# NVlabs/ODISE

Hardware: AMD Instinct MI355X
Metric: panoptic-inference images/sec @1024x1024 (higher is better)
Workload: dtype f16

## Files before the change

### include/odise_hip_tools.h

```cpp
#ifndef ODISE_HIP_TOOLS_H
#define ODISE_HIP_TOOLS_H

#include "odise_hip.h"

#ifdef __cplusplus
extern "C" {
#endif

int odise_hip_sizeof_gemm_desc(void);
int odise_hip_sizeof_conv_desc(void);
int odise_hip_sizeof_attn_desc(void);
int odise_hip_sizeof_post_desc(void);
int odise_hip_sizeof_infer_desc(void);

int odise_hip_gemm_forced(odise_hip_ctx* ctx, const odise_gemm_desc* d, int tile, int splitk);
int odise_hip_conv2d_forced(odise_hip_ctx* ctx, const odise_conv_desc* d, int tile, int splitk);
int odise_hip_last_tile(void);
int odise_hip_gemm_ln(odise_hip_ctx* ctx, const odise_gemm_desc* d, const float* part, int parts, float inv_c, float eps, const float* colsum,
                      float* final_out, const float* fin, const float* rowsum, float* stats_out);
int odise_hip_conv2d_gn_forced(odise_hip_ctx* ctx, const odise_conv_desc* d, int tile, int splitk, const float* gamma, const float* beta,
                               int groups, float eps, int act, void* y_norm, float* stats_scratch, int* stats_blocks);
int odise_hip_gemm_debug(int flags);

int odise_hip_post_generic(int on);
int odise_hip_sem_tile(int tile);
int odise_hip_gn_tuning(int chunk_factor, int fold_in_apply);
int odise_hip_msda_unfused(int on);
int odise_hip_msda_fused_forward(odise_hip_ctx* ctx, const void* value, const float* off, const float* aw, const int* hs3, const int* ws3, int B, int M, int fused,
                                 void* out, float* loc_scratch, float* w_scratch);

int odise_hip_stage_timeline(odise_hip_ctx* ctx, int on);
int odise_hip_stage_timeline_read(odise_hip_ctx* ctx, char* names, int names_cap, float* gpu_ms, double* host_ms, int cap, int* n);

int odise_hip_prefetch_stats(odise_hip_ctx* ctx, int* enqueued, int* hits, int* dropped, int* failed);

int odise_hip_launch_log(odise_hip_ctx* ctx, int on);
int odise_hip_launch_log_read(odise_hip_ctx* ctx, int* out6, int cap, int* n);

int odise_hip_set_lanes(odise_hip_ctx* ctx, int lanes);

int odise_hip_backbone_maps(odise_hip_ctx* ctx, float** out4, int* shape_bchw4x4);

int odise_hip_mfma_probe(odise_hip_ctx* ctx, float* host_out);

int odise_hip_maskclip_token_mask(odise_hip_ctx* ctx, const void* logits_f16, void* out_u8, int B, int Q, int h, int w, int S, int patch, int T,
                                  int64_t ldm, int plain);
#ifdef __cplusplus
}
#endif
#endif
```

### odise_amd/csrc/engine.cpp

```cpp
#include <stdlib.h>

#include "engine.h"

#include <string.h>

namespace odise {

void unet_destroy(ModelStore* ms);
void extractor_destroy(ModelStore* ms);
void maskgen_destroy(ModelStore* ms);
void classify_destroy(ModelStore* ms);

ModelStore* store_of(odise_hip_ctx* ctx) {
    if (!ctx->models) ctx->models = new ModelStore();
    return (ModelStore*)ctx->models;
}

void free_allocs(std::vector<void*>& owned) {
    if (owned.empty()) return;
    (void)hipDeviceSynchronize();
    for (void* p : owned) (void)hipFree(p);
    owned.clear();
}

// ... 195 lines not shown
    if (x.c != w.cin_pad) {
        set_error("conv: input has %d channels, weight expects %d", x.c, w.cin_pad);
        return ODISE_ERR_ARG;
    }
    if (pad < 0) pad = w.k / 2;
    if (pad_t < 0) pad_t = pad;
    if (pad_l < 0) pad_l = pad;
    const int hin = upsample ? 2 * x.h : x.h, win = upsample ? 2 * x.w : x.w;
    if (oh < 0) oh = (hin + 2 * pad - w.k) / stride + 1;
    if (ow < 0) ow = (win + 2 * pad - w.k) / stride + 1;
    if (!y.p) ODISE_TRY(alloc(y, x.n, oh, ow, w.cout));
    odise_conv_desc d;
    memset(&d, 0, sizeof(d));
    d.N = x.n; d.H = x.h; d.W = x.w; d.Cin = x.c;
    d.Cout = w.cout; d.KH = w.k; d.KW = w.k; d.stride = stride; d.pad_t = pad_t; d.pad_l = pad_l; d.OH = oh; d.OW = ow;
    d.upsample2x = upsample ? 1 : 0;
    d.X = x.p; d.Wt = w.w; d.Y = y.p; d.y_dtype = ODISE_F16;
    d.bias = w.b;
    d.residual = residual ? residual->p : nullptr;
    d.per_image_add = per_image_add;
    d.per_image_add_ld = pia_ld;
    d.act = act;
    ms->macs += (double)x.n * oh * ow * w.cout * w.k * w.k * w.cin;
    y.gn_blocks = 0;
#ifdef ODISE_TOOLS
    if (y.gn_part && getenv("ODISE_NO_GN_FUSION")) return odise_hip_conv2d(ctx, &d);
#endif
    if (y.gn_part) return conv_forced(ctx, &d, -1, 0, y.gn_part, &y.gn_blocks);
    return odise_hip_conv2d(ctx, &d);
}

int Exec::alloc_gn_stats(Act& a) {
    const int64_t blocks = ceil_div((int64_t)a.h * a.w, 64);
    a.gn_part = (float*)alloc_bytes((size_t)a.n * blocks * a.c * 2 * sizeof(float));
    a.gn_blocks = 0;
    return a.gn_part ? ODISE_OK : ODISE_ERR_NOMEM;
}

int Exec::linear(const f16* x, int64_t M, const LinW& w, f16* y, int act, const f16* residual, bool geglu) {
    odise_gemm_desc d;
    memset(&d, 0, sizeof(d));
    d.M = (int)M; d.N = w.out; d.K = w.in;
    d.A = x; d.lda = w.in;
    d.W = w.w; d.ldw = w.in;
    d.C = y; d.ldc = geglu ? w.out / 2 : w.out; d.c_dtype = ODISE_F16;
    d.bias_n = w.b;
    d.residual = residual; d.ldr = d.ldc;
    d.act = act; d.geglu = geglu ? 1 : 0; d.alpha = 1.f; d.batch = 1;
    return gemm(d);
}

int Exec::group_norm(const Act& x, const NormW& w, Act& y, float eps, int act) {
    if (!y.p) ODISE_TRY(alloc(y, x.n, x.h, x.w, x.c));
    if (x.gn_part && x.gn_blocks > 0)
        return group_norm_from_colpart(ctx, x.p, y.p, w.g, w.b, x.n, x.h * x.w, x.c, 32, eps, act, x.gn_part, x.gn_blocks);
    return odise_hip_group_norm(ctx, x.p, y.p, w.g, w.b, x.n, x.h * x.w, x.c, 32, eps, act);
}

int Exec::layer_norm(const f16* x, f16* y, int64_t rows, const NormW& w, float eps) {
    return odise_hip_layer_norm(ctx, x, y, w.g, w.b, (int)rows, w.c, eps);
}

}

using namespace odise;

extern "C" int odise_hip_load_weight(odise_hip_ctx* ctx, const char* name, const float* host_data, const int64_t* shape, int ndim) {
    ODISE_REQUIRE(ctx && name && host_data && (ndim == 0 || shape), "load_weight: null argument");
    ODISE_REQUIRE(ndim >= 0 && ndim <= 4, "load_weight: rank %d not in [0,4]", ndim);
    ModelStore* ms = store_of(ctx);
    HostTensor t;
    int64_t n = 1;
    for (int i = 0; i < ndim; ++i) {
        ODISE_REQUIRE(shape[i] >= 0, "load_weight: negative dim");
        t.shape.push_back(shape[i]);
        n *= shape[i];
    }
    t.data.assign(host_data, host_data + n);
    ms->host[std::string(name)] = std::move(t);
    return ODISE_OK;
}

extern "C" int odise_hip_clear_host_weights(odise_hip_ctx* ctx) {
    ODISE_REQUIRE(ctx, "clear_host_weights: null context");
    store_of(ctx)->host.clear();
    return ODISE_OK;
}
```

### odise_amd/csrc/engine.h

```cpp
#pragma once
#include <map>
#include <utility>
#include <string>
#include <vector>

#include "common.h"

namespace odise {

struct HostTensor {
    std::vector<float> data;
    std::vector<int64_t> shape;
    int64_t numel() const {
        int64_t n = 1;
        for (auto s : shape) n *= s;
        return n;
    }
};

struct Arena {
    char* base = nullptr;
    size_t cap = 0, off = 0, peak = 0;
    void* alloc(size_t bytes) {
        off = (off + 255) & ~(size_t)255;
// ... 34 lines not shown
};

struct UNetModel;

struct EncoderOut {
    Act tap0, tap1;
    Act xt, zdec;
};
struct PrefetchKey {
    int B = 0, layout = 0;
    std::vector<const void*> images;
    std::vector<int> hw;
    bool operator==(const PrefetchKey& o) const { return B == o.B && layout == o.layout && images == o.images && hw == o.hw; }
};
struct Prefetch {
    bool has_pending = false, has_ready = false;
    PrefetchKey pending, ready;
    int ready_slot = 0;
    EncoderOut out;
    int crops = 0;
    bool use_now = false;
    int n_enqueued = 0, n_hits = 0, n_dropped = 0, n_failed = 0;
    Arena arena[2];
};

struct ClipKV {
    void* buf = nullptr;
    size_t cap = 0;
    f16* qk = nullptr;
    f16* vt = nullptr;
    f16* cls = nullptr;
    int B = 0, TP = 0, layers = 0, width = 0;
    size_t qk_stride = 0, vt_stride = 0;
    int64_t ldvt = 0;
    const float* plan_image = nullptr;
    int plan_B = 0, plan_H = 0, plan_W = 0;
    bool planned = false, ready = false, on_lane2 = false;
};

struct ModelStore {
    std::map<std::string, HostTensor> host;
    std::vector<void*> dev_allocs;
    std::vector<void*>* alloc_sink = nullptr;
    void track(void* p) { (alloc_sink ? *alloc_sink : dev_allocs).push_back(p); }
    Arena arena;
    Arena arena2;
    Prefetch pf;
    ClipKV mclip;
    UNetModel* unet = nullptr;
    struct ExtractorModel* extractor = nullptr;
    struct MaskGenModel* maskgen = nullptr;
    struct ClassifyModel* classify = nullptr;
    double macs = 0.0;
};

ModelStore* store_of(odise_hip_ctx* ctx);
struct AllocScope {
    ModelStore* ms;
    std::vector<void*>* prev;
    AllocScope(ModelStore* m, std::vector<void*>& owned) : ms(m), prev(m->alloc_sink) { m->alloc_sink = &owned; }
    ~AllocScope() { ms->alloc_sink = prev; }
};
void free_allocs(std::vector<void*>& owned);

struct Packer {
    odise_hip_ctx* ctx;
    ModelStore* ms;
    std::string prefix;
    std::string missing;

    const HostTensor* find(const std::string& key);
    int upload(const void* host, size_t bytes, void** dev);
    int conv(const std::string& key, ConvW& out, bool bias = true);
    int linear(const std::string& key, LinW& out, bool bias = true);
    int norm(const std::string& key, NormW& out);
    int vec_f32(const std::string& key, float** out, int64_t expect);
};

struct Exec {
    odise_hip_ctx* ctx;
    ModelStore* ms;
    int alloc(Act& a, int n, int h, int w, int c);
    int alloc_gn_stats(Act& a);
    void* alloc_bytes(size_t bytes);

    int conv(const Act& x, const ConvW& w, Act& y, int stride = 1, int pad = -1, bool upsample = false, const Act* residual = nullptr,
             const float* per_image_add = nullptr, int64_t pia_ld = 0, int act = ODISE_ACT_NONE, int pad_t = -1, int pad_l = -1,
             int oh = -1, int ow = -1);
    int linear(const f16* x, int64_t M, const LinW& w, f16* y, int act = ODISE_ACT_NONE, const f16* residual = nullptr,
               bool geglu = false);
    int group_norm(const Act& x, const NormW& w, Act& y, float eps, int act);
    int layer_norm(const f16* x, f16* y, int64_t rows, const NormW& w, float eps);
    int gemm(const odise_gemm_desc& d);
    int attention(const odise_attn_desc& d);
};


int ensure_lane2(odise_hip_ctx* ctx, ModelStore* ms, size_t arena_bytes);
struct Lane2 {
    odise_hip_ctx* ctx;
    ModelStore* ms;
    hipStream_t s0;
    void* w0;
    Lane2(odise_hip_ctx* c, ModelStore* m) : ctx(c), ms(m), s0(c->stream), w0(c->ws) {
        ctx->stream = ctx->stream2;
        ctx->ws = ctx->ws2;
// ... 137 lines not shown
```

### odise_amd/csrc/gemm.hip

```cpp
#include "common.h"
#include <stdlib.h>
#include <type_traits>

#ifdef ODISE_TOOLS
#define ODISE_ABLATE(g, bit) ((g).dbg & (bit))
#else
#define ODISE_ABLATE(g, bit) false
#endif

namespace odise {

struct GemmEpi {
    void* C;
    int64_t ldc;
    int c_dtype;
    const float* bias_n;
    const float* bias_m;
    const float* scale_m;
    const f16* residual;
    int64_t ldr;
    const float* rowgroup_add;
    int rows_per_group;
    int64_t ldg;
    int act;
// ... 771 lines not shown
        }
        __syncthreads();
        if (stats) {
            float* red = reinterpret_cast<float*>(smem);
            if (lane < CHW) {
#pragma unroll
                for (int i = 0; i < 8; ++i) {
                    red[((wm * BN) + wn * WTN + lane * 8 + i) * 2 + 0] = s8[i];
                    red[((wm * BN) + wn * WTN + lane * 8 + i) * 2 + 1] = q8[i];
                }
            }
            __syncthreads();
            for (int c = threadIdx.x; c < BN; c += 64 * NWAVES) {
                float a = 0.f, bb = 0.f;
                for (int r = 0; r < WAVES_M; ++r) { a += red[(r * BN + c) * 2]; bb += red[(r * BN + c) * 2 + 1]; }
                if (n0 + c < g.N) {
                    float* o = e.gn_stats + ((int64_t)(m0 / BM) * g.N + n0 + c) * 2;
                    o[0] = a;
                    o[1] = bb;
                }
            }
        }
    }
}

template <int BM, int BN, int WAVES_M, int WAVES_N, int WG, bool HALO = false, bool STATS = false, bool PAIRS = true, int EW16 = 0, bool GEGLU_OK = false, int LDSB = 0>
__device__ __forceinline__ void gemm_epilogue(const GemmArgs& g, WaveAcc<BM, BN, WAVES_M, WAVES_N>& acc, char* smem, int m0, int n0, int z, int zb, bool split) {
    using FL = FragLayout;
    if constexpr (LDSB > 0 && WAVES_M * WAVES_N == 8 && (64 % ((BN / WAVES_N) / 8)) == 0) {
        if (g.epi.fast && !split && !g.epi.geglu && !g.epi_block && !ODISE_ABLATE(g, 8)) {
            gemm_epilogue_wave<BM, BN, WAVES_M, WAVES_N, HALO, STATS, GEGLU_OK, LDSB>(g, acc, smem, m0, n0, zb);
            return;
        }
    }
    if constexpr (EW16 > 0) {
        if (g.epi.f16path && !split && !ODISE_ABLATE(g, 8)) {
            if constexpr (GEGLU_OK) {
                if (g.epi.geglu) { gemm_epilogue_f16<BM, BN, WAVES_M, WAVES_N, EW16, HALO, false, true>(g, acc, smem, m0, n0, zb); return; }
            }
            if (!g.epi.geglu) { gemm_epilogue_f16<BM, BN, WAVES_M, WAVES_N, EW16, HALO, STATS, false>(g, acc, smem, m0, n0, zb); return; }
        }
    }
    constexpr int NT = 64 * WAVES_M * WAVES_N;
    constexpr int WTM = BM / WAVES_M, WTN = BN / WAVES_N;
    constexpr int TM = WTM / 32, TN = WTN / 32;
    constexpr int ROWS = WG * WTM;
    const int tid = threadIdx.x;
    const int lane = tid & 63;
    const int wave = tid >> 6;
    const int wm = wave / WAVES_N, wn = wave % WAVES_N;
    constexpr int LDS_LD = BN + 4;
    constexpr int CH = BN / 8;
    float* stg = reinterpret_cast<float*>(smem);
    const bool stats = STATS && (NT % CH == 0) && g.epi.gn_stats != nullptr && !split;
    float s8[8], q8[8];
#pragma unroll
    for (int i = 0; i < 8; ++i) s8[i] = q8[i] = 0.f;
    constexpr int LPR = (BN * 2 + 127) / 128;
    constexpr int NPF = (BM * LPR + NT - 1) / NT;
    unsigned pf[NPF];
    const bool prefetch = g.epi.residual != nullptr && !split && !ODISE_ABLATE(g, 64);
    if (prefetch) {
#pragma unroll
        for (int i = 0; i < NPF; ++i) {
            const int li = tid + i * NT;
            const int rt = li / LPR, seg = li - rt * LPR;
            int m = m0 + rt;
            if (HALO) {
                const int patch = m0 / BM;
                const int per_img = g.cg.halo_tx * g.cg.halo_ty;
                const int img = patch / per_img, pr = patch - img * per_img;
                const int oy = (pr / g.cg.halo_tx) * 16 + (rt >> 4), ox = (pr % g.cg.halo_tx) * 16 + (rt & 15);
                m = (oy < g.cg.OH && ox < g.cg.OW) ? (img * g.cg.OH + oy) * g.cg.OW + ox : g.M;
            }
            pf[i] = 0u;
            if (rt < BM && m < g.M && n0 + seg * 64 + 2 <= g.N)
                pf[i] = *reinterpret_cast<const unsigned*>(g.epi.residual + (int64_t)zb * g.epi.strideR + (int64_t)m * g.epi.ldr + n0 + seg * 64);
        }
        asm volatile("" ::: "memory");
    }
#pragma unroll
    for (int gp = 0; gp < WAVES_M / WG; ++gp) {
        if (gp > 0) lds_barrier();
        if (wm / WG == gp) {
#pragma unroll
            for (int p = 0; p < TM; ++p)
#pragma unroll
                for (int j = 0; j < TN; ++j) {
#pragma unroll
                    for (int rr = 0; rr < FL::NR; ++rr) {
                        const int row = (wm % WG) * WTM + p * 32 + FL::row(lane, rr);
#pragma unroll
                        for (int q = 0; q < FL::NC; ++q) {
                            const int col = wn * WTN + j * 32 + FL::col(lane, q);
                            const int r0 = 4 * (rr * FL::NC + q);
                            *reinterpret_cast<float4*>(&stg[row * LDS_LD + col]) =
                                make_float4(acc_get(acc, p, j, r0), acc_get(acc, p, j, r0 + 1), acc_get(acc, p, j, r0 + 2), acc_get(acc, p, j, r0 + 3));
                        }
                    }
                }
        }
        lds_barrier();
        if (gp == 0 && prefetch) {
#pragma unroll
            for (int i = 0; i < NPF; ++i) asm volatile("" ::"v"(pf[i]));
        }
        if constexpr ((NT % CH == 0) && ((ROWS * CH) % NT == 0)) {
            if (g.epi.fast && !split && n0 + BN <= g.N && !ODISE_ABLATE(g, 8)) {
                constexpr int IT = (ROWS * CH) / NT, RSTEP = NT / CH;
                constexpr int U = (IT % 2 == 0 && PAIRS && !STATS && !HALO) ? 2 : 1;
// ... 70 lines not shown
#pragma unroll
                            for (int i = 0; i < 8; ++i) b[i] += bm;
                        }
#pragma unroll
                        for (int i = 0; i < 8; ++i) v[i] = v[i] * alpha + b[i];
                        if (e.geglu) {
                            float o[4];
#pragma unroll
                            for (int i = 0; i < 4; ++i) o[i] = v[2 * i] * gelu_erf(v[2 * i + 1]);
                            const int64_t off = (int64_t)zb * e.strideC + (int64_t)m * e.ldc + (n >> 1);
                            if (e.c_dtype == ODISE_F16) {
                                f16x4 t;
#pragma unroll
                                for (int i = 0; i < 4; ++i) t[i] = (f16)o[i];
                                *reinterpret_cast<f16x4*>((f16*)e.C + off) = t;
                            } else {
                                *reinterpret_cast<float4*>((float*)e.C + off) = make_float4(o[0], o[1], o[2], o[3]);
                            }
                            continue;
                        }
                        if (e.act == ODISE_ACT_SILU) {
#pragma unroll
                            for (int i = 0; i < 8; ++i) v[i] = mul_sigmoid(v[i], v[i]);
                        } else if (e.act == ODISE_ACT_RELU) {
#pragma unroll
                            for (int i = 0; i < 8; ++i) v[i] = v[i] > 0.f ? v[i] : 0.f;
                        } else if (e.act == ODISE_ACT_QUICKGELU) {
#pragma unroll
                            for (int i = 0; i < 8; ++i) v[i] = mul_sigmoid(v[i], 1.702f * v[i]);
                        } else if (e.act == ODISE_ACT_GELU) {
#pragma unroll
                            for (int i = 0; i < 8; ++i) v[i] = gelu_erf(v[i]);
                        }
                        const int64_t off = (int64_t)zb * e.strideC + (int64_t)m * e.ldc + n;
                        if (e.c_dtype == ODISE_F16) {
                            f16x8 t;
#pragma unroll
                            for (int i = 0; i < 8; ++i) t[i] = (f16)(v[i] + (float)rr[u][i]);
                            *reinterpret_cast<f16x8*>((f16*)e.C + off) = t;
                            if (stats) {
#pragma unroll
                                for (int i = 0; i < 8; ++i) { const float r = (float)t[i]; s8[i] += r; q8[i] += r * r; }
                            }
                        } else {
                            float* c = (float*)e.C + off;
                            *reinterpret_cast<float4*>(c) = make_float4(v[0] + (float)rr[u][0], v[1] + (float)rr[u][1], v[2] + (float)rr[u][2], v[3] + (float)rr[u][3]);
                            *reinterpret_cast<float4*>(c + 4) = make_float4(v[4] + (float)rr[u][4], v[5] + (float)rr[u][5], v[6] + (float)rr[u][6], v[7] + (float)rr[u][7]);
                        }
                    }
                }
                continue;
            }
        }
        for (int c = tid; c < ROWS * CH; c += NT) {
            const int row = c / CH;
            const int c8 = c - row * CH;
            int m = m0 + gp * ROWS + row;
            if (HALO) {
                const int rt = gp * ROWS + row;
                const int patch = m0 / BM;
                const int per_img = g.cg.halo_tx * g.cg.halo_ty;
                const int img = patch / per_img, pr = patch - img * per_img;
                const int oy = (pr / g.cg.halo_tx) * 16 + (rt >> 4), ox = (pr % g.cg.halo_tx) * 16 + (rt & 15);
                m = (oy < g.cg.OH && ox < g.cg.OW) ? (img * g.cg.OH + oy) * g.cg.OW + ox : g.M;
            }
            const int n = n0 + c8 * 8;
            if (m < g.M && n < g.N) {
                float v[8];
                const float4 t0 = *reinterpret_cast<const float4*>(&stg[row * LDS_LD + c8 * 8]);
                const float4 t1 = *reinterpret_cast<const float4*>(&stg[row * LDS_LD + c8 * 8 + 4]);
                v[0] = t0.x; v[1] = t0.y; v[2] = t0.z; v[3] = t0.w;
                v[4] = t1.x; v[5] = t1.y; v[6] = t1.z; v[7] = t1.w;
                if (split) {
                    float* w = g.ws + ((int64_t)z * g.M + m) * g.N + n;
                    const int nv = (g.N - n) < 8 ? (g.N - n) : 8;
                    if (nv == 8 && (g.N & 3) == 0) {
                        *reinterpret_cast<float4*>(w) = t0;
                        *reinterpret_cast<float4*>(w + 4) = t1;
                    } else {
                        for (int i = 0; i < nv; ++i) w[i] = v[i];
                    }
                } else if (!(ODISE_ABLATE(g, 8)) || v[0] == 12345.678f) {
                    if (g.epi.fast && n + 8 <= g.N) {
                        if (stats) {
                            float r8[8];
                            epi_fast8(g.epi, v, m, n, zb, r8);
#pragma unroll
                            for (int i = 0; i < 8; ++i) { s8[i] += r8[i]; q8[i] += r8[i] * r8[i]; }
                        } else {
                            epi_fast8(g.epi, v, m, n, zb);
                        }
                    } else {
                        epi_store8(g.epi, v, m, n, g.N, zb);
                    }
                }
            }
        }
    }
    if (stats) {
        constexpr int RL = NT / CH;
        lds_barrier();
        float* red = reinterpret_cast<float*>(smem);
        const int c8 = tid % CH, rl = tid / CH;
#pragma unroll
        for (int i = 0; i < 8; ++i) {
            red[((rl * BN) + c8 * 8 + i) * 2 + 0] = s8[i];
            red[((rl * BN) + c8 * 8 + i) * 2 + 1] = q8[i];
        }
        lds_barrier();
        for (int c = tid; c < BN; c += NT) {
            float a = 0.f, b = 0.f;
            for (int r = 0; r < RL; ++r) { a += red[(r * BN + c) * 2]; b += red[(r * BN + c) * 2 + 1]; }
            if (n0 + c < g.N) {
                float* o = g.epi.gn_stats + ((int64_t)(m0 / BM) * g.N + n0 + c) * 2;
                o[0] = a;
                o[1] = b;
            }
        }
    }
}

struct Frag {
    static constexpr int NSTEP = 2;
    static constexpr int PER = 2;
    static __device__ __forceinline__ int lrow(int lane) { return lane & 15; }
    static __device__ __forceinline__ int lk(int lane) { return lane >> 4; }
    static __device__ __forceinline__ int kslot(int st, int lk) { return st * 4 + lk; }
};
__device__ __forceinline__ void acc_zero(AccBlock& a) {
#pragma unroll
    for (int t = 0; t < 4; ++t) a[t] = f32x4{0.f, 0.f, 0.f, 0.f};
}
__device__ __forceinline__ void mma_step(AccBlock& acc, const f16x8 (&b)[2], const f16x8 (&a)[2]) {
#pragma unroll
    for (int rt = 0; rt < 2; ++rt)
#pragma unroll
        for (int ct = 0; ct < 2; ++ct) acc[rt * 2 + ct] = __builtin_amdgcn_mfma_f32_16x16x32_f16(b[ct], a[rt], acc[rt * 2 + ct], 0, 0, 0);
}

template <int BM, int BN, int WAVES_M, int WAVES_N, bool CONV>
__global__ void __launch_bounds__(64 * WAVES_M * WAVES_N) gemm_kernel(GemmArgs g) {
    constexpr int BK = 64;
    constexpr int NT = 64 * WAVES_M * WAVES_N;
    constexpr int WTM = BM / WAVES_M, WTN = BN / WAVES_N;
    constexpr int TM = WTM / 32, TN = WTN / 32;
    constexpr int RPI = NT / 8;
    constexpr int JA = BM / RPI, JB = BN / RPI;
    constexpr int STAGE_BYTES = (BM + BN) * BK * 2;
    static_assert(WTM % 32 == 0 && WTN % 32 == 0 && BM % RPI == 0 && BN % RPI == 0 && RPI % 16 == 0, "bad tile");
    extern __shared__ __attribute__((aligned(16))) char smem[];

    const int tid = threadIdx.x;
    const int lane = tid & 63;
    const int wave = tid >> 6;
    const int wm = wave / WAVES_N, wn = wave % WAVES_N;
    const int hi = lane >> 5, l31 = lane & 31;
    int bx, by;
    {
        const int nbx = gridDim.x, nb = gridDim.x * gridDim.y;
        const int bid = blockIdx.y * nbx + blockIdx.x;
// ... 1327 lines not shown
            if (sp > 1 && (size_t)sp * g.M * g.N * sizeof(float) > ctx->ws_bytes) break;
            const int per = is_halo_tile(t) ? (int)ceil_div(nk / 9, sp) * 9 : (int)ceil_div(nk, sp);
            const int eff_sp = (int)ceil_div(nk, per);
            const int64_t nblk = nb * eff_sp;
            const int64_t rounds = ceil_div(nblk, slots);
            const double fill_last = (double)(nblk - (rounds - 1) * slots) / (double)slots;
            double t_us = per * tc.t_ktile * ((double)(rounds - 1) + 0.55 + 0.45 * fill_last) + (double)rounds * tc.t_fixed;
            if (eff_sp > 1) t_us += 4.0 + ((2.0 * eff_sp * 4.0 + 2.0) * (double)g.M * g.N) / 6.0e6;
            if (t_us < best) { best = t_us; tile = t; best_split = eff_sp; }
        }
    }
    if (force_tile >= 0 && force_tile < kNumTiles && !(force_tile == kTile512x128 && !pp_ok) && !(is_halo_tile(force_tile) && !(halo_ok && pp_base)))
        tile = force_tile;
    g.splitk = 1;
    g.ktiles_per_split = nk;
    if (force_split > 0 && batch == 1) best_split = std::min(force_split, nk);
    if (best_split > 1 && batch == 1) {
        g.ktiles_per_split = is_halo_tile(tile) ? (int)ceil_div(nk / 9, best_split) * 9 : (int)ceil_div(nk, best_split);
        g.splitk = (int)ceil_div(nk, g.ktiles_per_split);
        ODISE_REQUIRE((size_t)g.splitk * g.M * g.N * sizeof(float) <= ctx->ws_bytes, "gemm: split-K workspace too small");
    }
    g_last_tile = tile | (best_split << 8);
    if (ctx->launch_log) launch_log_push(ctx, LaunchRec{(int)CONV, g.M, g.N, g.K, tile, g.splitk});
    if (flags & kFlagLaunchLog) {
        fprintf(stderr, "GEMMLOG conv=%d M=%d N=%d K=%d batch=%d cin=%d kh=%d h=%d w=%d stride=%d ups=%d tile=%d split=%d pp=%d\n", (int)CONV, g.M, g.N,
                g.K, batch, g.cg.Cin, g.cg.KH, g.cg.H, g.cg.W, g.cg.stride, g.cg.ups, tile, best_split, (int)pp_ok);
    }
    g.ws = (float*)ctx->ws;
    {
        const GemmEpi& e = g.epi;
        const int esz = e.c_dtype == ODISE_F16 ? 2 : 4;
        const int out_vec = (e.geglu ? 4 : 8) * esz;
        auto aligned = [](const void* p, int64_t ld_elems, int64_t stride_elems, int elem, int bytes) {
            return ((uintptr_t)p % bytes) == 0 && (ld_elems * elem) % bytes == 0 && (stride_elems * elem) % bytes == 0;
        };
        bool ok = aligned(e.C, e.ldc, e.strideC, esz, out_vec);
        ok = ok && (!e.residual || (!e.geglu && aligned(e.residual, e.ldr, e.strideR, 2, 16)));
        ok = ok && (!e.bias_n || ((uintptr_t)e.bias_n & 15) == 0);
        ok = ok && (!e.rowgroup_add || (((uintptr_t)e.rowgroup_add & 15) == 0 && e.ldg % 4 == 0));
        ok = ok && (!e.geglu || e.act == ODISE_ACT_NONE);
        g.epi.fast = ok ? 1 : 0;
        const int n_out = e.geglu ? g.N / 2 : g.N;
        g.epi.f16path = (ok && e.c_dtype == ODISE_F16 && g.N % 8 == 0 && n_out % 8 == 0 && aligned(e.C, e.ldc, e.strideC, 2, 16) &&
                         (!e.residual || aligned(e.residual, e.ldr, e.strideR, 2, 8))) ? 1 : 0;
    }
    if (g.epi.ln_part || g.epi.ln_final || g.epi.ln_stats_out) {
        ODISE_REQUIRE(!CONV && (tile == kTile256x256 || tile == kTile256x128) && g.splitk == 1 && g.epi.f16path && !g.epi.geglu && batch == 1 &&
                          (!g.epi.ln_stats_out || (tile == kTile256x256 && g.N % kLnPartCols == 0)),
                      "gemm_ln: M=%d N=%d K=%d cannot take the folded-LayerNorm path", g.M, g.N, g.K);
    }
    g.stats_blocks = 0;
    if (g.epi.gn_stats) {
        const int ohw = CONV ? g.cg.OH * g.cg.OW : 0;
        const bool pp2_used = (tile == kTile256x256) && pp_ok && ((flags & kFlagForcePP2) || (!(flags & kFlagNoPP2) && CONV));
        bool ok = CONV && g.splitk == 1 && g.epi.fast && g.N % 8 == 0 &&
                  (is_halo_tile(tile) || (tile == kTile512x128 && pp_ok && !(flags & kFlagForcePP2)) || pp2_used);
        if (ok && is_halo_tile(tile)) g.stats_blocks = g.cg.halo_tx * g.cg.halo_ty;
        else if (ok && ohw % kTileBM[tile] == 0) g.stats_blocks = ohw / kTileBM[tile];
        else ok = false;
        if (!ok) { g.epi.gn_stats = nullptr; g.stats_blocks = 0; }
    }
    g.zeros = (const f16*)ctx->zeros;
    g.epi_block = (flags & kFlagBlockEpilogue) ? 1 : 0;
#ifdef ODISE_TOOLS
    static const int freeze_k = (getenv("ODISE_GEMM_FREEZE_K") ? 16 : 0) | (getenv("ODISE_NO_RES_PREFETCH") ? 64 : 0);
    g.dbg = g_gemm_debug | freeze_k;
#else
    g.dbg = 0;
#endif
    if (is_halo_tile(tile)) {
        g.cg.chunk_major = 1;
        if (tile == kTileHalo128x4) return launch_conv3_halo4<128>(ctx, g);
        return tile == kTileHalo256 ? launch_conv3_halo<256, 2>(ctx, g) : launch_conv3_halo<128, 1>(ctx, g);
    }
    g.cg.halo_tx = g.cg.halo_ty = 0;
    const bool pp2_auto = !(flags & kFlagNoPP2) && ((CONV && tile != kTile512x128) || (!CONV && blocks(tile) * (g.splitk > 1 ? g.splitk : 1) <= 2 * cus));
    if (has_pingpong_form(tile) && pp_ok && ((flags & kFlagForcePP2) || pp2_auto)) {
        if (tile == kTile512x128) return launch_gemm_pp2<512, 128, 1, 2, CONV>(ctx, g, batch);
        if (tile == kTile256x320) return launch_gemm_pp2<256, 320, 2, 1, CONV>(ctx, g, batch);
        return launch_gemm_pp2<256, 256, 2, 2, CONV>(ctx, g, batch);
    }
    if (has_pingpong_form(tile) && pp_ok) {
        if (tile == kTile512x128) return launch_gemm_pp<512, 128, 1, 2, CONV>(ctx, g, batch);
        if (tile == kTile256x320) return launch_gemm_pp<256, 320, 2, 1, CONV>(ctx, g, batch);
        return launch_gemm_pp<256, 256, 2, 2, CONV>(ctx, g, batch);
    }
    switch (tile) {
        case kTile128x128: return launch_gemm_t<128, 128, 2, 2, CONV>(ctx, g, batch);
        case kTile64x128: return launch_gemm_t<64, 128, 2, 2, CONV>(ctx, g, batch);
        case kTile256x320: return launch_gemm_t<256, 320, 4, 2, CONV>(ctx, g, batch);
        case kTile256x256: return launch_gemm_t<256, 256, 4, 2, CONV>(ctx, g, batch);
        case kTile256x128: return launch_gemm_t<256, 128, 4, 2, CONV>(ctx, g, batch);
        default: return launch_gemm_t<64, 64, 2, 2, CONV>(ctx, g, batch);
    }
}

int conv_forced(odise_hip_ctx* ctx, const odise_conv_desc* d, int force_tile, int force_split, float* gn_stats = nullptr, int* stats_blocks = nullptr);

int gemm_forced(odise_hip_ctx* ctx, const odise_gemm_desc* d, int force_tile, int force_split, const LnEpi* ln) {
    ODISE_REQUIRE(ctx && d, "gemm: null argument");
    ODISE_REQUIRE(d->M >= 0 && d->N >= 0 && d->K > 0, "gemm: bad dims M=%d N=%d K=%d", d->M, d->N, d->K);
    if (d->M == 0 || d->N == 0) return ODISE_OK;
    ODISE_REQUIRE(d->K % 8 == 0, "gemm: K=%d must be a multiple of 8", d->K);
    ODISE_REQUIRE(d->lda % 8 == 0 && d->ldw % 8 == 0, "gemm: lda/ldw must be multiples of 8 (16-byte rows)");
    ODISE_REQUIRE(((uintptr_t)d->A & 15) == 0 && ((uintptr_t)d->W & 15) == 0, "gemm: A/W must be 16-byte aligned");
    ODISE_REQUIRE(d->A && d->W && d->C, "gemm: null device pointer");
    ODISE_REQUIRE(d->c_dtype == ODISE_F16 || d->c_dtype == ODISE_F32, "gemm: bad c_dtype");
// ... 102 lines not shown
```

### odise_amd/csrc/unet.cpp

```cpp
#include <math.h>
#include <string.h>

#include "engine.h"

namespace odise {

struct ResBlockW {
    NormW n1, n2;
    ConvW c1, c2, skip;
    bool has_skip = false;
    int cin = 0, cout = 0;
    int emb_off = 0;
};

struct STBlockW {
    int c = 0;
    NormW gn, ln1, ln2, ln3;
    LinW proj_in, proj_out;
    LinW qk1, v1, o1;
    LinW q2, k2, v2, o2;
    LinW ff1, ff2;
    int ctx_slot = 0;
};

struct UBlock {
    bool has_res = false, has_st = false, has_down = false, has_up = false, is_conv_in = false;
    ResBlockW res;
    STBlockW st;
    ConvW conv;
};

struct UNetModel {
    std::vector<void*> owned;
    bool built = false;
    LinW te0, te2;
    LinW emb_all;
    std::vector<UBlock> in_blocks, out_blocks;
    ResBlockW mid_r1, mid_r2;
    STBlockW mid_st;
    int n_ctx_slots = 0;
    int emb_total = 0;
    int mc = 320, ted = 1280, cdim = 768;
    int cached_t = -1, cached_B = 0;
    f16* temb_in = nullptr;
    bool use_graph = false;
    hipGraphExec_t graph_exec = nullptr;
    int graph_B = 0, graph_h = 0, graph_w = 0;
    const void *graph_x = nullptr, *graph_ctx = nullptr, *graph_ce = nullptr, *graph_arena = nullptr;
    Act taps[4];
    double last_macs = 0.0;
};

const Act* unet_taps(ModelStore* ms) { return ms->unet ? ms->unet->taps : nullptr; }
double unet_last_macs(ModelStore* ms) { return ms->unet ? ms->unet->last_macs : 0.0; }

void unet_destroy(ModelStore* ms) {
    if (!ms->unet) return;
    if (ms->unet->graph_exec) (void)hipGraphExecDestroy(ms->unet->graph_exec);
    free_allocs(ms->unet->owned);
    if (ms->unet->temb_in) { (void)hipDeviceSynchronize(); (void)hipFree(ms->unet->temb_in); }
    delete ms->unet;
    ms->unet = nullptr;
}

static int build_res(Packer& pk, const std::string& key, ResBlockW& r, std::vector<const HostTensor*>& emb_w,
                     std::vector<const HostTensor*>& emb_b, int& emb_total, int pk_ted) {
    ODISE_TRY(pk.norm(key + ".in_layers.0", r.n1));
    ODISE_TRY(pk.conv(key + ".in_layers.2", r.c1));
    ODISE_TRY(pk.norm(key + ".out_layers.0", r.n2));
    ODISE_TRY(pk.conv(key + ".out_layers.3", r.c2));
    r.cin = r.c1.cin;
    r.cout = r.c1.cout;
    r.has_skip = pk.find(key + ".skip_connection.weight") != nullptr;
    if (r.has_skip) ODISE_TRY(pk.conv(key + ".skip_connection", r.skip));
    else if (r.cin != r.cout) {
        set_error("unet: '%s' changes channels %d->%d but has no skip_connection", key.c_str(), r.cin, r.cout);
        return ODISE_ERR_STATE;
    }
    const HostTensor* w = pk.find(key + ".emb_layers.1.weight");
    const HostTensor* b = pk.find(key + ".emb_layers.1.bias");
    if (!w || !b || w->shape.size() != 2 || w->shape[0] != r.cout || w->shape[1] != pk_ted) {
        set_error("unet: bad or missing '%s.emb_layers.1'", key.c_str());
        return ODISE_ERR_STATE;
    }
    r.emb_off = emb_total;
    emb_total += r.cout;
    emb_w.push_back(w);
    emb_b.push_back(b);
    return ODISE_OK;
}

static int build_st(Packer& pk, const std::string& key, STBlockW& s, int& n_slots) {
    ODISE_TRY(pk.norm(key + ".norm", s.gn));
    s.c = s.gn.c;
    ODISE_TRY(pk.linear(key + ".proj_in", s.proj_in));
    ODISE_TRY(pk.linear(key + ".proj_out", s.proj_out));
    const std::string tb = key + ".transformer_blocks.0";
    ODISE_TRY(pk.norm(tb + ".norm1", s.ln1));
    ODISE_TRY(pk.norm(tb + ".norm2", s.ln2));
    ODISE_TRY(pk.norm(tb + ".norm3", s.ln3));
    const HostTensor* wq = pk.find(tb + ".attn1.to_q.weight");
    const HostTensor* wk = pk.find(tb + ".attn1.to_k.weight");
    if (!wq || !wk || wq->numel() != (int64_t)s.c * s.c || wk->numel() != (int64_t)s.c * s.c) {
// ... 78 lines not shown
        }
        u->in_blocks.push_back(b);
    }
    ODISE_TRY(build_res(pk, "middle_block.0", u->mid_r1, emb_w, emb_b, u->emb_total, u->ted));
    ODISE_TRY(build_st(pk, "middle_block.1", u->mid_st, u->n_ctx_slots));
    ODISE_TRY(build_res(pk, "middle_block.2", u->mid_r2, emb_w, emb_b, u->emb_total, u->ted));
    for (int i = 0; i < 11; ++i) {
        UBlock b;
        const std::string k = "output_blocks." + std::to_string(i);
        b.has_res = true;
        ODISE_TRY(build_res(pk, k + ".0", b.res, emb_w, emb_b, u->emb_total, u->ted));
        int next = 1;
        if (pk.find(k + ".1.norm.weight")) {
            b.has_st = true;
            ODISE_TRY(build_st(pk, k + ".1", b.st, u->n_ctx_slots));
            next = 2;
        }
        if (pk.find(k + "." + std::to_string(next) + ".conv.weight")) {
            b.has_up = true;
            ODISE_TRY(pk.conv(k + "." + std::to_string(next) + ".conv", b.conv));
        }
        u->out_blocks.push_back(b);
    }
    u->cdim = u->mid_st.k2.in;
    {
        const size_t ted = (size_t)u->ted;
        std::vector<f16> w((size_t)u->emb_total * ted);
        std::vector<float> bvec((size_t)u->emb_total);
        size_t row = 0;
        for (size_t i = 0; i < emb_w.size(); ++i) {
            const size_t rows = (size_t)emb_w[i]->shape[0];
            for (size_t j = 0; j < rows * ted; ++j) w[row * ted + j] = (f16)emb_w[i]->data[j];
            for (size_t j = 0; j < rows; ++j) bvec[row + j] = emb_b[i]->data[j];
            row += rows;
        }
        u->emb_all.in = (int)ted; u->emb_all.out = u->emb_total;
        ODISE_TRY(pk.upload(w.data(), w.size() * sizeof(f16), (void**)&u->emb_all.w));
        ODISE_TRY(pk.upload(bvec.data(), bvec.size() * sizeof(float), (void**)&u->emb_all.b));
    }
    u->built = true;
    return ODISE_OK;
}

struct UNetRun {
    Exec ex;
    UNetModel* u;
    int B;
    const float* emb_out;
    f16* ctx16;
    std::vector<f16*> ctxK;
    std::vector<f16*> ctxVt;
};

static int run_res(UNetRun& r, const ResBlockW& w, const Act& x, Act& out) {
    Exec& ex = r.ex;
    ODISE_TRY(ex.alloc(out, x.n, x.h, x.w, w.cout));
    const size_t mk = ex.ms->arena.mark();
    Act t1, hcur, t2, sk;
    ODISE_TRY(ex.group_norm(x, w.n1, t1, 1e-5f, ODISE_ACT_SILU));
    ODISE_TRY(ex.conv(t1, w.c1, hcur, 1, 1, false, nullptr, r.emb_out + w.emb_off, r.u->emb_total));
    ODISE_TRY(ex.group_norm(hcur, w.n2, t2, 1e-5f, ODISE_ACT_SILU));
    const Act* resid = &x;
    if (w.has_skip) {
        ODISE_TRY(ex.conv(x, w.skip, sk, 1, 0));
        resid = &sk;
    }
    ODISE_TRY(ex.conv(t2, w.c2, out, 1, 1, false, resid));
    ex.ms->arena.release(mk);
    return ODISE_OK;
}

static int run_st(UNetRun& r, const STBlockW& w, const Act& x, Act& out) {
    Exec& ex = r.ex;
    const int C = w.c, heads = 8, D = C / heads;
    const int64_t HW = (int64_t)x.h * x.w, M = x.pixels();
    ODISE_TRY(ex.alloc(out, x.n, x.h, x.w, C));
    const size_t mk = ex.ms->arena.mark();
    Act t;
    ODISE_TRY(ex.group_norm(x, w.gn, t, 1e-6f, ODISE_ACT_NONE));
    f16* hs = (f16*)ex.alloc_bytes((size_t)M * C * 2);
    f16* nrm = (f16*)ex.alloc_bytes((size_t)M * C * 2);
    f16* qk = (f16*)ex.alloc_bytes((size_t)M * 2 * C * 2);
    const int64_t ldvt = round_up(HW, 8);
    f16* vt = (f16*)ex.alloc_bytes((size_t)x.n * C * ldvt * 2);
    f16* att = (f16*)ex.alloc_bytes((size_t)M * C * 2);
    f16* hs2 = (f16*)ex.alloc_bytes((size_t)M * C * 2);
    f16* ffh = (f16*)ex.alloc_bytes((size_t)M * 4 * C * 2);
    if (!hs || !nrm || !qk || !vt || !att || !hs2 || !ffh) return ODISE_ERR_NOMEM;
    ODISE_TRY(ex.linear(t.p, M, w.proj_in, hs));
    ODISE_TRY(ex.layer_norm(hs, nrm, M, w.ln1, 1e-5f));
    ODISE_TRY(ex.linear(nrm, M, w.qk1, qk));
    {
        odise_gemm_desc d;
        memset(&d, 0, sizeof(d));
        d.M = C; d.N = (int)HW; d.K = C;
        d.A = w.v1.w; d.lda = C; d.strideA = 0;
        d.W = nrm; d.ldw = C; d.strideW = HW * C;
        d.C = vt; d.ldc = ldvt; d.strideC = (int64_t)C * ldvt; d.c_dtype = ODISE_F16;
        d.alpha = 1.f; d.batch = x.n;
        ODISE_TRY(ex.gemm(d));
        odise_attn_desc a;
        memset(&a, 0, sizeof(a));
        a.B = x.n; a.H = heads; a.Lq = (int)HW; a.Lk = (int)HW; a.D = D;
        a.Q = qk; a.ldq = 2 * C; a.strideQ = HW * 2 * C;
        a.K = qk + C; a.ldk = 2 * C; a.strideK = HW * 2 * C;
        a.Vt = vt; a.ldvt = ldvt; a.strideVt = (int64_t)C * ldvt;
        a.O = att; a.ldo = C; a.strideO = HW * C;
        a.scale = 1.0f / sqrtf((float)D);
        ODISE_TRY(ex.attention(a));
    }
    ODISE_TRY(ex.linear(att, M, w.o1, hs2, ODISE_ACT_NONE, hs));
    ODISE_TRY(ex.layer_norm(hs2, nrm, M, w.ln2, 1e-5f));
// ... 50 lines not shown
        memset(&d, 0, sizeof(d));
        d.M = B; d.N = u->ted; d.K = u->ted;
        d.A = te_h; d.lda = u->ted; d.W = u->te2.w; d.ldw = u->ted;
        d.C = emb_silu; d.ldc = u->ted; d.c_dtype = ODISE_F16;
        d.bias_n = u->te2.b;
        d.rowgroup_add = cond_emb; d.rows_per_group = 1; d.ldg = u->ted;
        d.act = ODISE_ACT_SILU; d.alpha = 1.f; d.batch = 1;
        ODISE_TRY(ex.gemm(d));
        memset(&d, 0, sizeof(d));
        d.M = B; d.N = u->emb_total; d.K = u->ted;
        d.A = emb_silu; d.lda = u->ted; d.W = u->emb_all.w; d.ldw = u->ted;
        d.C = emb_out; d.ldc = u->emb_total; d.c_dtype = ODISE_F32;
        d.bias_n = u->emb_all.b; d.alpha = 1.f; d.batch = 1;
        ODISE_TRY(ex.gemm(d));
    }
    r.emb_out = emb_out;

    r.ctx16 = (f16*)ex.alloc_bytes((size_t)B * 77 * u->cdim * 2);
    if (!r.ctx16) return ODISE_ERR_NOMEM;
    ODISE_TRY(odise_hip_cast_f32_to_f16(ctx, context, r.ctx16, (size_t)B * 77 * u->cdim));
    r.ctxK.assign(u->n_ctx_slots, nullptr);
    r.ctxVt.assign(u->n_ctx_slots, nullptr);
    auto prep_ctx = [&](const STBlockW& s) -> int {
        const int C = s.c;
        f16* k = (f16*)ex.alloc_bytes((size_t)B * 77 * C * 2);
        f16* vt = (f16*)ex.alloc_bytes((size_t)B * C * 80 * 2);
        if (!k || !vt) return ODISE_ERR_NOMEM;
        ODISE_TRY(ex.linear(r.ctx16, (int64_t)B * 77, s.k2, k));
        odise_gemm_desc d;
        memset(&d, 0, sizeof(d));
        d.M = C; d.N = 77; d.K = u->cdim;
        d.A = s.v2.w; d.lda = u->cdim; d.strideA = 0;
        d.W = r.ctx16; d.ldw = u->cdim; d.strideW = 77 * (int64_t)u->cdim;
        d.C = vt; d.ldc = 80; d.strideC = (int64_t)C * 80; d.c_dtype = ODISE_F16;
        d.alpha = 1.f; d.batch = B;
        ODISE_TRY(ex.gemm(d));
        r.ctxK[s.ctx_slot] = k;
        r.ctxVt[s.ctx_slot] = vt;
        return ODISE_OK;
    };
    for (auto& b : u->in_blocks)
        if (b.has_st) ODISE_TRY(prep_ctx(b.st));
    ODISE_TRY(prep_ctx(u->mid_st));
    for (auto& b : u->out_blocks)
        if (b.has_st) ODISE_TRY(prep_ctx(b.st));

    Act x0;
    if (x_nhwc) {
        x0.p = const_cast<f16*>(x_nhwc); x0.n = B; x0.h = h; x0.w = w; x0.c = 8;
    } else {
        ODISE_TRY(ex.alloc(x0, B, h, w, 8));
        ODISE_TRY(odise_hip_nchw_f32_to_nhwc_f16(ctx, x_t, x0.p, B, 4, h, w, 8));
    }
    std::vector<Act> hs;
    Act cur = x0;
    for (auto& b : u->in_blocks) {
        Act nxt;
        if (b.is_conv_in) {
            ODISE_TRY(ex.conv(cur, b.conv, nxt, 1, 1));
        } else if (b.has_down) {
            ODISE_TRY(ex.conv(cur, b.conv, nxt, 2, 1));
        } else {
            ODISE_TRY(run_res(r, b.res, cur, nxt));
            if (b.has_st) {
                Act o2;
                ODISE_TRY(run_st(r, b.st, nxt, o2));
                nxt = o2;
            }
        }
        hs.push_back(nxt);
        cur = nxt;
    }
    {
        Act a, b2, c;
        ODISE_TRY(run_res(r, u->mid_r1, cur, a));
        ODISE_TRY(run_st(r, u->mid_st, a, b2));
        ODISE_TRY(run_res(r, u->mid_r2, b2, c));
        cur = c;
    }
    int tap_i = 0;
    for (int i = 0; i < 12; ++i) {
        const Act skip = hs.back();
        hs.pop_back();
        Act cat;
        ODISE_TRY(ex.alloc(cat, cur.n, cur.h, cur.w, cur.c + skip.c));
        ODISE_TRY(odise_hip_concat_channels(ctx, cur.p, skip.p, cat.p, (size_t)cur.pixels(), cur.c, skip.c));
        if (i == 2 || i == 5 || i == 8 || i == 11) u->taps[tap_i++] = cat;
        if (i == 11) break;
        const UBlock& b = u->out_blocks[i];
        Act nxt;
        ODISE_TRY(run_res(r, b.res, cat, nxt));
        if (b.has_st) {
            Act o2;
            ODISE_TRY(run_st(r, b.st, nxt, o2));
            nxt = o2;
        }
        if (b.has_up) {
            Act o3;
            ODISE_TRY(ex.conv(nxt, b.conv, o3, 1, 1, true));
            nxt = o3;
        }
        cur = nxt;
    }
    u->last_macs = ms->macs;
    return ODISE_OK;
}

int unet_prepare_timestep(odise_hip_ctx* ctx, ModelStore* ms, UNetModel* u, int B, int t) {
    if (u->cached_t != t || u->cached_B < B) {
        std::vector<f16> te((size_t)B * u->mc);
        const int half = u->mc / 2;
        for (int i = 0; i < half; ++i) {
            const double f = exp(-log(10000.0) * i / (double)half);
            for (int b = 0; b < B; ++b) {
                te[(size_t)b * u->mc + i] = (f16)(float)cos((double)t * f);
                te[(size_t)b * u->mc + half + i] = (f16)(float)sin((double)t * f);
            }
        }
        ODISE_CHECK_HIP(hipDeviceSynchronize());
        if (u->temb_in) ODISE_CHECK_HIP(hipFree(u->temb_in));
        u->temb_in = nullptr;
        ODISE_CHECK_HIP(hipMalloc((void**)&u->temb_in, te.size() * 2));
        ODISE_CHECK_HIP(hipMemcpy(u->temb_in, te.data(), te.size() * 2, hipMemcpyHostToDevice));
        u->cached_t = t;
        u->cached_B = B;
        if (u->graph_exec) { (void)hipGraphExecDestroy(u->graph_exec); u->graph_exec = nullptr; }
    }
    return ODISE_OK;
}

static int unet_forward(odise_hip_ctx* ctx, const float* x_t, const float* context, const float* cond_emb, int B, int h, int w, int t) {
    ModelStore* ms = store_of(ctx);
    UNetModel* u = ms->unet;
    if (!u || !u->built) {
        set_error("unet_features: call odise_hip_unet_build first");
        return ODISE_ERR_STATE;
    }
    ODISE_REQUIRE(B >= 1 && h >= 8 && w >= 8 && h % 8 == 0 && w % 8 == 0, "unet_features: latent %dx%d (batch %d) must be multiples of 8", h, w, B);
    ODISE_REQUIRE(x_t && context, "unet_features: null device pointer");
    ODISE_TRY(unet_prepare_timestep(ctx, ms, u, B, t));
    const size_t per_crop = (size_t)640 << 20;
    const double scale = ((double)h * w) / (64.0 * 64.0);
    ODISE_TRY(ensure_arena(ctx, ms, (size_t)(per_crop * (scale < 0.25 ? 0.25 : scale)) * B + ((size_t)64 << 20)));

    if (!u->use_graph) return unet_launch(ctx, ms, u, x_t, nullptr, context, cond_emb, B, h, w, true);

    const bool same = u->graph_exec && u->graph_B == B && u->graph_h == h && u->graph_w == w && u->graph_x == x_t &&
                      u->graph_ctx == context && u->graph_ce == cond_emb && u->graph_arena == ms->arena.base;
    if (!same) {
        if (u->graph_exec) { (void)hipGraphExecDestroy(u->graph_exec); u->graph_exec = nullptr; }
        hipGraph_t graph = nullptr;
        ODISE_CHECK_HIP(hipStreamBeginCapture(ctx->stream, hipStreamCaptureModeThreadLocal));
        const int rc = unet_launch(ctx, ms, u, x_t, nullptr, context, cond_emb, B, h, w, true);
        const hipError_t e = hipStreamEndCapture(ctx->stream, &graph);
        if (rc != ODISE_OK) {
            if (graph) (void)hipGraphDestroy(graph);
            return rc;
// ... 6 lines not shown
    }
    ODISE_CHECK_HIP(hipGraphLaunch(u->graph_exec, ctx->stream));
    return ODISE_OK;
}

}

using namespace odise;

extern "C" int odise_hip_unet_build(odise_hip_ctx* ctx) {
    ODISE_REQUIRE(ctx, "unet_build: null context");
    ODISE_CHECK_HIP(hipSetDevice(ctx->device));
    return unet_build(ctx, "");
}

extern "C" int odise_hip_unet_use_graph(odise_hip_ctx* ctx, int enable) {
    ODISE_REQUIRE(ctx, "unet_use_graph: null context");
    ModelStore* ms = store_of(ctx);
    if (!ms->unet) {
        set_error("unet_use_graph: call odise_hip_unet_build first");
        return ODISE_ERR_STATE;
    }
    ms->unet->use_graph = enable != 0;
    return ODISE_OK;
}

extern "C" int odise_hip_unet_features_nhwc(odise_hip_ctx* ctx, const float* x_t, const float* context, const float* cond_emb, int B,
                                            int h, int w, int t, void** taps4) {
    ODISE_REQUIRE(ctx, "unet_features: null context");
    ODISE_CHECK_HIP(hipSetDevice(ctx->device));
    ODISE_TRY(unet_forward(ctx, x_t, context, cond_emb, B, h, w, t));
    if (taps4) {
        ModelStore* ms = store_of(ctx);
        for (int i = 0; i < 4; ++i) taps4[i] = ms->unet->taps[i].p;
    }
    return ODISE_OK;
}

extern "C" int odise_hip_unet_features(odise_hip_ctx* ctx, const float* x_t, const float* context, const float* cond_emb, int B, int h,
                                       int w, int t, float* tap_u2, float* tap_u5, float* tap_u8, float* tap_u11) {
    ODISE_REQUIRE(ctx, "unet_features: null context");
    ODISE_CHECK_HIP(hipSetDevice(ctx->device));
    ODISE_TRY(unet_forward(ctx, x_t, context, cond_emb, B, h, w, t));
    ModelStore* ms = store_of(ctx);
    float* outs[4] = {tap_u2, tap_u5, tap_u8, tap_u11};
    for (int i = 0; i < 4; ++i) {
        if (!outs[i]) continue;
        const Act& a = ms->unet->taps[i];
        ODISE_TRY(odise_hip_nhwc_f16_to_nchw_f32(ctx, a.p, outs[i], a.n, a.c, a.h, a.w));
    }
    return ODISE_OK;
}

extern "C" int odise_hip_unet_last_macs(odise_hip_ctx* ctx, double* macs) {
    ODISE_REQUIRE(ctx && macs, "unet_last_macs: null argument");
    ModelStore* ms = store_of(ctx);
    *macs = ms->unet ? ms->unet->last_macs : 0.0;
    return ODISE_OK;
}
```

Measured before the change: 53.04.

## Fuse GroupNorm statistics into UNet conv epilogues across more blocks

Pre-allocates GroupNorm partial-statistics buffers on conv outputs in UNet res blocks, conv_in/downsample convs and mid blocks, so the following GroupNorm can use the fused column-partial path instead of a standalone reduction pass. The GEMM epilogue gains an LDS-backed statistics accumulator for tiles whose thread count does not divide the channel chunking, and the 256x320 tile becomes eligible for stats fusion. This is meant to remove separate GN reduction kernels and their extra reads of activations. The cost is more LDS traffic in the epilogue and added fold logic. It also adds counters and a tool API for fused versus standalone norm counts.

New measurement: 52.96. About the same (-0.2%).

```diff
diff --git a/include/odise_hip_tools.h b/include/odise_hip_tools.h
--- a/include/odise_hip_tools.h
+++ b/include/odise_hip_tools.h
@@ -20,6 +20,7 @@
                       float* final_out, const float* fin, const float* rowsum, float* stats_out);
 int odise_hip_conv2d_gn_forced(odise_hip_ctx* ctx, const odise_conv_desc* d, int tile, int splitk, const float* gamma, const float* beta,
                                int groups, float eps, int act, void* y_norm, float* stats_scratch, int* stats_blocks);
+int odise_hip_unet_norm_counts(odise_hip_ctx* ctx, int* gn_fused, int* gn_standalone);
 int odise_hip_gemm_debug(int flags);
 
 int odise_hip_post_generic(int on);
diff --git a/odise_amd/csrc/engine.cpp b/odise_amd/csrc/engine.cpp
--- a/odise_amd/csrc/engine.cpp
+++ b/odise_amd/csrc/engine.cpp
@@ -271,6 +271,7 @@
 
 int Exec::group_norm(const Act& x, const NormW& w, Act& y, float eps, int act) {
     if (!y.p) ODISE_TRY(alloc(y, x.n, x.h, x.w, x.c));
+    ++(x.gn_part && x.gn_blocks > 0 ? ms->gn_fused : ms->gn_alone);
     if (x.gn_part && x.gn_blocks > 0)
         return group_norm_from_colpart(ctx, x.p, y.p, w.g, w.b, x.n, x.h * x.w, x.c, 32, eps, act, x.gn_part, x.gn_blocks);
     return odise_hip_group_norm(ctx, x.p, y.p, w.g, w.b, x.n, x.h * x.w, x.c, 32, eps, act);
diff --git a/odise_amd/csrc/engine.h b/odise_amd/csrc/engine.h
--- a/odise_amd/csrc/engine.h
+++ b/odise_amd/csrc/engine.h
@@ -110,6 +110,7 @@
     struct MaskGenModel* maskgen = nullptr;
     struct ClassifyModel* classify = nullptr;
     double macs = 0.0;
+    int gn_fused = 0, gn_alone = 0;
 };
 
 ModelStore* store_of(odise_hip_ctx* ctx);
diff --git a/odise_amd/csrc/gemm.hip b/odise_amd/csrc/gemm.hip
--- a/odise_amd/csrc/gemm.hip
+++ b/odise_amd/csrc/gemm.hip
@@ -847,10 +847,18 @@
     constexpr int LDS_LD = BN + 4;
     constexpr int CH = BN / 8;
     float* stg = reinterpret_cast<float*>(smem);
-    const bool stats = STATS && (NT % CH == 0) && g.epi.gn_stats != nullptr && !split;
+    constexpr int NTS = (STATS && NT % CH != 0) ? (NT / CH) * CH : NT;
+    const bool stats = STATS && g.epi.gn_stats != nullptr && !split;
     float s8[8], q8[8];
 #pragma unroll
     for (int i = 0; i < 8; ++i) s8[i] = q8[i] = 0.f;
+    constexpr bool STATS_LDS = STATS && (NT % CH != 0);
+    static_assert(!STATS_LDS || (ROWS * LDS_LD + 16 * NTS) * (int)sizeof(float) <= LDSB, "no room for the statistics behind the staging rows");
+    float4* const sacc = reinterpret_cast<float4*>(stg + ROWS * LDS_LD) + (tid < NTS ? tid : 0);
+    if (STATS_LDS && stats && tid < NTS) {
+#pragma unroll
+        for (int j = 0; j < 4; ++j) sacc[j * NTS] = make_float4(0.f, 0.f, 0.f, 0.f);
+    }
     constexpr int LPR = (BN * 2 + 127) / 128;
     constexpr int NPF = (BM * LPR + NT - 1) / NT;
     unsigned pf[NPF];
@@ -1027,7 +1035,7 @@
                 continue;
             }
         }
-        for (int c = tid; c < ROWS * CH; c += NT) {
+        for (int c = tid < NTS ? tid : ROWS * CH; c < ROWS * CH; c += NTS) {
             const int row = c / CH;
             const int c8 = c - row * CH;
             int m = m0 + gp * ROWS + row;
@@ -1060,8 +1068,17 @@
                         if (stats) {
                             float r8[8];
                             epi_fast8(g.epi, v, m, n, zb, r8);
-#pragma unroll
-                            for (int i = 0; i < 8; ++i) { s8[i] += r8[i]; q8[i] += r8[i] * r8[i]; }
+                            if constexpr (STATS_LDS) {
+                                float4 a0 = sacc[0], a1 = sacc[NTS], b0 = sacc[2 * NTS], b1 = sacc[3 * NTS];
+                                a0.x += r8[0]; a0.y += r8[1]; a0.z += r8[2]; a0.w += r8[3];
+                                a1.x += r8[4]; a1.y += r8[5]; a1.z += r8[6]; a1.w += r8[7];
+                                b0.x += r8[0] * r8[0]; b0.y += r8[1] * r8[1]; b0.z += r8[2] * r8[2]; b0.w += r8[3] * r8[3];
+                                b1.x += r8[4] * r8[4]; b1.y += r8[5] * r8[5]; b1.z += r8[6] * r8[6]; b1.w += r8[7] * r8[7];
+                                sacc[0] = a0; sacc[NTS] = a1; sacc[2 * NTS] = b0; sacc[3 * NTS] = b1;
+                            } else {
+#pragma unroll
+                                for (int i = 0; i < 8; ++i) { s8[i] += r8[i]; q8[i] += r8[i] * r8[i]; }
+                            }
                         } else {
                             epi_fast8(g.epi, v, m, n, zb);
                         }
@@ -1072,15 +1089,23 @@
             }
         }
     }
+    if (STATS_LDS && stats && tid < NTS) {
+        const float4 a0 = sacc[0], a1 = sacc[NTS], b0 = sacc[2 * NTS], b1 = sacc[3 * NTS];
+        s8[0] = a0.x; s8[1] = a0.y; s8[2] = a0.z; s8[3] = a0.w; s8[4] = a1.x; s8[5] = a1.y; s8[6] = a1.z; s8[7] = a1.w;
+        q8[0] = b0.x; q8[1] = b0.y; q8[2] = b0.z; q8[3] = b0.w; q8[4] = b1.x; q8[5] = b1.y; q8[6] = b1.z; q8[7] = b1.w;
+    }
     if (stats) {
-        constexpr int RL = NT / CH;
+        constexpr int RL = NTS / CH;
+        static_assert(!STATS || RL * BN * 2 <= ROWS * LDS_LD, "the statistics fold outgrows the staging buffer");
         lds_barrier();
         float* red = reinterpret_cast<float*>(smem);
         const int c8 = tid % CH, rl = tid / CH;
-#pragma unroll
-        for (int i = 0; i < 8; ++i) {
-            red[((rl * BN) + c8 * 8 + i) * 2 + 0] = s8[i];
-            red[((rl * BN) + c8 * 8 + i) * 2 + 1] = q8[i];
+        if (tid < NTS) {
+#pragma unroll
+            for (int i = 0; i < 8; ++i) {
+                red[((rl * BN) + c8 * 8 + i) * 2 + 0] = s8[i];
+                red[((rl * BN) + c8 * 8 + i) * 2 + 1] = q8[i];
+            }
         }
         lds_barrier();
         for (int c = tid; c < BN; c += NT) {
@@ -2514,7 +2539,7 @@
     g.stats_blocks = 0;
     if (g.epi.gn_stats) {
         const int ohw = CONV ? g.cg.OH * g.cg.OW : 0;
-        const bool pp2_used = (tile == kTile256x256) && pp_ok && ((flags & kFlagForcePP2) || (!(flags & kFlagNoPP2) && CONV));
+        const bool pp2_used = (tile == kTile256x256 || tile == kTile256x320) && pp_ok && ((flags & kFlagForcePP2) || (!(flags & kFlagNoPP2) && CONV));
         bool ok = CONV && g.splitk == 1 && g.epi.fast && g.N % 8 == 0 &&
                   (is_halo_tile(tile) || (tile == kTile512x128 && pp_ok && !(flags & kFlagForcePP2)) || pp2_used);
         if (ok && is_halo_tile(tile)) g.stats_blocks = g.cg.halo_tx * g.cg.halo_ty;
diff --git a/odise_amd/csrc/unet.cpp b/odise_amd/csrc/unet.cpp
--- a/odise_amd/csrc/unet.cpp
+++ b/odise_amd/csrc/unet.cpp
@@ -49,6 +49,7 @@
     const void *graph_x = nullptr, *graph_ctx = nullptr, *graph_ce = nullptr, *graph_arena = nullptr;
     Act taps[4];
     double last_macs = 0.0;
+    int last_gn_fused = 0, last_gn_alone = 0;
 };
 
 const Act* unet_taps(ModelStore* ms) { return ms->unet ? ms->unet->taps : nullptr; }
@@ -233,12 +234,15 @@
     std::vector<f16*> ctxVt;
 };
 
-static int run_res(UNetRun& r, const ResBlockW& w, const Act& x, Act& out) {
+static int run_res(UNetRun& r, const ResBlockW& w, const Act& x, Act& out, bool out_to_norm) {
     Exec& ex = r.ex;
     ODISE_TRY(ex.alloc(out, x.n, x.h, x.w, w.cout));
+    if (out_to_norm) ODISE_TRY(ex.alloc_gn_stats(out));
     const size_t mk = ex.ms->arena.mark();
     Act t1, hcur, t2, sk;
     ODISE_TRY(ex.group_norm(x, w.n1, t1, 1e-5f, ODISE_ACT_SILU));
+    ODISE_TRY(ex.alloc(hcur, x.n, x.h, x.w, w.cout));
+    ODISE_TRY(ex.alloc_gn_stats(hcur));
     ODISE_TRY(ex.conv(t1, w.c1, hcur, 1, 1, false, nullptr, r.emb_out + w.emb_off, r.u->emb_total));
     ODISE_TRY(ex.group_norm(hcur, w.n2, t2, 1e-5f, ODISE_ACT_SILU));
     const Act* resid = &x;
@@ -395,16 +399,21 @@
         ODISE_TRY(ex.alloc(x0, B, h, w, 8));
         ODISE_TRY(odise_hip_nchw_f32_to_nhwc_f16(ctx, x_t, x0.p, B, 4, h, w, 8));
     }
+    const int gn_fused0 = ms->gn_fused, gn_alone0 = ms->gn_alone;
     std::vector<Act> hs;
     Act cur = x0;
-    for (auto& b : u->in_blocks) {
+    for (size_t bi = 0; bi < u->in_blocks.size(); ++bi) {
+        const UBlock& b = u->in_blocks[bi];
+        const bool next_is_res = bi + 1 < u->in_blocks.size() ? u->in_blocks[bi + 1].has_res : true;
         Act nxt;
-        if (b.is_conv_in) {
-            ODISE_TRY(ex.conv(cur, b.conv, nxt, 1, 1));
-        } else if (b.has_down) {
-            ODISE_TRY(ex.conv(cur, b.conv, nxt, 2, 1));
+        if (b.is_conv_in || b.has_down) {
+            const int stride = b.has_down ? 2 : 1;
+            const int oh = (cur.h + 2 - b.conv.k) / stride + 1, ow = (cur.w + 2 - b.conv.k) / stride + 1;
+            ODISE_TRY(ex.alloc(nxt, cur.n, oh, ow, b.conv.cout));
+            if (next_is_res) ODISE_TRY(ex.alloc_gn_stats(nxt));
+            ODISE_TRY(ex.conv(cur, b.conv, nxt, stride, 1));
         } else {
-            ODISE_TRY(run_res(r, b.res, cur, nxt));
+            ODISE_TRY(run_res(r, b.res, cur, nxt, b.has_st || next_is_res));
             if (b.has_st) {
                 Act o2;
                 ODISE_TRY(run_st(r, b.st, nxt, o2));
@@ -416,9 +425,9 @@
     }
     {
         Act a, b2, c;
-        ODISE_TRY(run_res(r, u->mid_r1, cur, a));
+        ODISE_TRY(run_res(r, u->mid_r1, cur, a, true));
         ODISE_TRY(run_st(r, u->mid_st, a, b2));
-        ODISE_TRY(run_res(r, u->mid_r2, b2, c));
+        ODISE_TRY(run_res(r, u->mid_r2, b2, c, false));
         cur = c;
     }
     int tap_i = 0;
@@ -432,7 +441,7 @@
         if (i == 11) break;
         const UBlock& b = u->out_blocks[i];
         Act nxt;
-        ODISE_TRY(run_res(r, b.res, cat, nxt));
+        ODISE_TRY(run_res(r, b.res, cat, nxt, b.has_st));
         if (b.has_st) {
             Act o2;
             ODISE_TRY(run_st(r, b.st, nxt, o2));
@@ -446,6 +455,8 @@
         cur = nxt;
     }
     u->last_macs = ms->macs;
+    u->last_gn_fused = ms->gn_fused - gn_fused0;
+    u->last_gn_alone = ms->gn_alone - gn_alone0;
     return ODISE_OK;
 }
 
@@ -558,6 +569,14 @@
     return ODISE_OK;
 }
 
+extern "C" int odise_hip_unet_norm_counts(odise_hip_ctx* ctx, int* gn_fused, int* gn_standalone) {
+    ODISE_REQUIRE(ctx && gn_fused && gn_standalone, "unet_norm_counts: null argument");
+    ModelStore* ms = store_of(ctx);
+    *gn_fused = ms->unet ? ms->unet->last_gn_fused : 0;
+    *gn_standalone = ms->unet ? ms->unet->last_gn_alone : 0;
+    return ODISE_OK;
+}
+
 extern "C" int odise_hip_unet_last_macs(odise_hip_ctx* ctx, double* macs) {
     ODISE_REQUIRE(ctx && macs, "unet_last_macs: null argument");
     ModelStore* ms = store_of(ctx);
```
